# JuliaMolSim/Molly.jl

Hardware: AMD Instinct MI355X
Metric: ns_per_day (higher is better)
Workload: dtype f32; 1 GPU; 1M-atom LJ fluid (argon, rho=21.1/nm3), cubic PBC, DistanceCutoff 1.0 nm, r_list 1.2 nm, dt 2 fs, VelocityVerlet, remove_CM_motion=1; integrator=vv, n_atoms=1000000, rebuild_every=10, parallelism=single domain, block_atoms=256, j_split=2, pairs_half_list=75841147

## Files before the change

molly.jl_amd/csrc/kernels.h:

```cpp
#pragma once
#include <type_traits>
#include "pass_plan.h"
#include "physics.h"
#include "halo_xfer.h"
#include "philox.h"

namespace mhip {

enum { FLAG_MINIMG = 0, FLAG_OVERFLOW = 1, FLAG_MAX_TILE = 2, FLAG_MAX_ROWS = 3, FLAG_NAN = 4, FLAG_TOTAL_ROWS = 5, FLAG_MAX_CELLS = 6, FLAG_MAX_DISP2 = 7, FLAG_MAX_V2 = 8, N_FLAGS = 10 };
enum { OVF_TILE = 1, OVF_ROWS = 2, OVF_BOXCELLS = 4, OVF_SLOT = 8 };

constexpr int MAX_BOX_CELLS = 8192;
constexpr uint32_t XL_EXCLUDED = 1u << 30, XL_SPECIAL = 1u << 31, XL_INDEX = (1u << 30) - 1u;

constexpr int SLOT_MAX_SCALED = 16383;
__host__ __device__ inline uint32_t entry_slot(uint32_t e, int sh) { return sh ? (e >> sh) : (e & 0x7fffu); }
__host__ __device__ inline uint32_t entry_special(uint32_t e, int sh) { return sh ? 0u : (e >> 15); }
__host__ __device__ inline uint32_t make_entry(uint32_t slot, uint32_t sp, int sh) { return sh ? (slot << sh) : (slot | (sp << 15)); }

template <class T> __device__ inline int cell_coord(T x, int d, const GridP<T>& G) {
    T rel = G.periodic[d] ? x : x - G.origin[d];
    int c = (int)M<T>::floor(rel * G.inv_cs[d]);
    return min(max(c, 0), G.nc[d] - 1);
}
// ... 1039 lines not shown
[[maybe_unused]] static __device__ inline void halo_tail(const HaloStep& H, const double* cm_part, int n_part) {
    const int lane = threadIdx.x & 63;
    double a[4] = {0, 0, 0, 0};
    if (cm_part) for (int q = lane; q < n_part; q += 64) for (int c = 0; c < 4; ++c) a[c] += __hip_atomic_load(&cm_part[4 * (int64_t)q + c], __ATOMIC_RELAXED, __HIP_MEMORY_SCOPE_AGENT);
#pragma unroll
    for (int o = 32; o > 0; o >>= 1) for (int c = 0; c < 4; ++c) a[c] += __shfl_xor(a[c], o, 64);
    if (lane < 4) H.cm_all[lane] = lane == 0 ? a[0] : lane == 1 ? a[1] : lane == 2 ? a[2] : a[3];
    for (int q = lane; q < H.n_peers * H.cm_rows; q += 64) {
        const int r = q % H.cm_rows;
        float* d = H.cm_dst[q] + (int64_t)H.parity_send * H.half_stride;
        for (int c = 0; c < 3; ++c) {
            const int i = 3 * r + c;
            const unsigned long long bits = (unsigned long long)__double_as_longlong(i < 2 ? a[0] : i < 4 ? a[1] : i < 6 ? a[2] : a[3]);
            const float w = i < 8 ? __uint_as_float((uint32_t)((i & 1) ? bits >> 32 : bits)) : 0.f;
            __hip_atomic_store(d + c, w, __ATOMIC_RELAXED, __HIP_MEMORY_SCOPE_SYSTEM);
        }
    }
    __threadfence_system();
    if (lane < H.n_peers) xfer_store_release(H.ann[lane] + (size_t)H.parity_send * XFER_MAX_RANKS, H.seq_send);
    if (lane == 0) __hip_atomic_store(H.done, 0u, __ATOMIC_RELAXED, __HIP_MEMORY_SCOPE_AGENT);
}

template <class T> struct ForceArgs {
    GridP<T> G;
    InterP<T> I;
    int64_t n_owned;
    int BI, BI_shift, JS, T_cap, T_lds, R_cap, n_blocks, blocks_per_xcd;
    const typename Vec<T>::T4* pos;
    const typename Vec<T>::T2* lj;
    const int32_t* tile_idx;
    const int32_t* tile_cnt;
    const uint2* nbr;
    const int32_t* wave_rows;
    const typename Vec<T>::T4* blk_center;
    typename Vec<T>::T4* frc;
    double* pe_part;
    uint2* nbr_dst; int32_t* rows_dst; const typename Vec<T>::T4* pos_snap; float* blk_disp2; T r_prune2;
    int32_t* tile_idx_dst; int32_t* tile_cnt_dst; int mark_off;
    typename Vec<T>::T4* snap_dst;
    int any_special;
    int soa;
    int eshift;
    uint16_t* cnt_dst;
    const int32_t* blk_ghost; int part;
    int level_pairs;
    unsigned long long* dbg;
    const double* cm_fin_in; int cm_fin_n; double* cm_fin_out;
    typename Vec<T>::T4* vel; typename Vec<T>::T4* pos_next; T dt, dt2;
    const double* cm_in; int cm_n; unsigned long long* cm_pub; uint32_t step_seq; double* cm_out;
    float* trk_part; const typename Vec<T>::T4* snap_a; const typename Vec<T>::T4* snap_b;
    HaloStep H;
    const int32_t* orig; StochP<T> S;
};
[[maybe_unused]] static __device__ inline void step_cm_publish(const double* __restrict__ part, int n_part, unsigned long long* pub, uint32_t seq, unsigned char* smem) {
    double (*sh_pub)[4] = reinterpret_cast<double (*)[4]>(smem);
    double a[4] = {0, 0, 0, 0};
    for (int q = threadIdx.x; q < n_part; q += blockDim.x) { const double* p = part + 4 * (int64_t)q; a[0] += p[0]; a[1] += p[1]; a[2] += p[2]; a[3] += p[3]; }
#pragma unroll
    for (int o = 32; o > 0; o >>= 1) for (int c = 0; c < 4; ++c) a[c] += __shfl_xor(a[c], o, 64);
    if ((threadIdx.x & 63) == 0) for (int c = 0; c < 4; ++c) sh_pub[threadIdx.x >> 6][c] = a[c];
    __syncthreads();
    if (threadIdx.x < 3) {
        double t = 0, m = 0;
        for (int q = 0; q < (int)(blockDim.x >> 6); ++q) { t += sh_pub[q][threadIdx.x]; m += sh_pub[q][3]; }
        const float vc = (float)(t / m);
        __hip_atomic_store(&pub[threadIdx.x], (unsigned long long)__float_as_uint(vc) | ((unsigned long long)seq << 32), __ATOMIC_RELAXED, __HIP_MEMORY_SCOPE_AGENT);
    }
}
[[maybe_unused]] static __device__ inline void cm_finalize_in_block(const double* __restrict__ part, int n_part, double* out4, unsigned char* smem) {
    double a[4] = {0, 0, 0, 0};
    for (int q = threadIdx.x; q < n_part; q += blockDim.x) { const double* p = part + 4 * (int64_t)q; a[0] += p[0]; a[1] += p[1]; a[2] += p[2]; a[3] += p[3]; }
#pragma unroll
    for (int o = 32; o > 0; o >>= 1) for (int c = 0; c < 4; ++c) a[c] += __shfl_xor(a[c], o, 64);
    double* sh = reinterpret_cast<double*>(smem);
    if ((threadIdx.x & 63) == 0) for (int c = 0; c < 4; ++c) sh[4 * (threadIdx.x >> 6) + c] = a[c];
    __syncthreads();
    if (threadIdx.x < 4) { double t = 0; for (int q = 0; q < (int)(blockDim.x >> 6); ++q) t += sh[4 * q + threadIdx.x]; out4[threadIdx.x] = t; }
    __syncthreads();
}

#ifndef MHIP_FAST_MIN_WAVES
#define MHIP_FAST_MIN_WAVES 8
#endif
#ifndef MHIP_SB
#define MHIP_SB 4
#endif
template <class T, int LJM, int COULM, bool ENERGY, bool MINIMG, bool SEG, bool PRUNE>
constexpr int force_min_waves() { return (std::is_same<T, float>::value && LJM == LJ_DIST_UNIFORM && COULM == MHIP_COUL_NONE && !ENERGY && !MINIMG && !SEG && !PRUNE) ? MHIP_FAST_MIN_WAVES : 1; }

template <class T, int LJM, int COULM, bool ENERGY, bool MINIMG, bool SEG, bool PRUNE, int SOA_STRIDE = 4097, bool STEP = false, bool HALO = false, bool LANG = false>
__global__ void __launch_bounds__(BlockLimits<T>::max_threads, (force_min_waves<T, LJM, COULM, ENERGY, MINIMG, SEG, PRUNE>()))
k_forces(ForceArgs<T> A) {
    static_assert(!HALO || (STEP && std::is_same<T, float>::value), "the ghosted form exists for the fused fp32 step only");
    static_assert(!LANG || (STEP && !HALO), "the Langevin update rides in the fused single-domain step only");
    using T4 = typename Vec<T>::T4;
    using T2 = typename Vec<T>::T2;
    constexpr bool PER_ATOM_LJ = (LJM == LJ_DIST || LJM == LJ_GENERIC);
    extern __shared__ __align__(32) unsigned char smem[];
    const GridP<T>& G = A.G;
    int wg = blockIdx.x;
    if constexpr (STEP) {
        if (wg == 0) {
            if constexpr (HALO) { if (A.cm_in) halo_cm_publish(A.H, A.cm_pub, A.step_seq, smem); }
            else if (A.cm_in) step_cm_publish(A.cm_in, A.cm_n, A.cm_pub, A.step_seq, smem);
            return;
        }
        --wg;
    }
    int b = (wg & 7) * A.blocks_per_xcd + (wg >> 3);
    [[maybe_unused]] int hflags = 0;
    if constexpr (HALO) { b = A.H.order[wg]; if (b < 0) return; hflags = A.H.flags[b]; }
    else {
        if (b >= A.n_blocks) return;
        if (A.part != 0 && (A.blk_ghost[b] != 0) != (A.part == 2)) return;
    }
    const int tid = threadIdx.x, nthr = blockDim.x;
    [[maybe_unused]] auto stamp = [&](int k) {
        if constexpr (MHIP_STAMPS != 0 && !PRUNE) {
            if (A.dbg && (tid & 63) == 0) { unsigned long long* d = A.dbg + ((size_t)b * (nthr >> 6) + (tid >> 6)) * 8; d[k] = __builtin_readcyclecounter(); d[4 + k] = wall_clock64(); }
        }
    };
    stamp(0);
    const int tile_n = A.tile_cnt[b];
    T4* l_pos = reinterpret_cast<T4*>(smem);
    T2* l_lj = reinterpret_cast<T2*>(l_pos + (A.T_lds + 1));
    const T4 ctr = A.blk_center[b];
    constexpr bool MAY_SCALE = std::is_same<T, float>::value && LJM == LJ_DIST_UNIFORM && COULM == MHIP_COUL_NONE;
    const int esh = MAY_SCALE ? A.eshift : 0;

    auto localise = [&](T4 p, auto tri_tag) -> T4 {
        if constexpr (!MINIMG) local_xyz_t<decltype(tri_tag)::value>(p.x, p.y, p.z, ctr, G);
        return p;
    };
    constexpr bool NO_TRI = std::is_same<T, float>::value && LJM == LJ_DIST_UNIFORM && COULM == MHIP_COUL_NONE && !ENERGY;
    const bool tri_local = !MINIMG && !NO_TRI && G.tri_grid;
    const int li = tid & (A.BI - 1), js = tid >> A.BI_shift;
    const int64_t si = (int64_t)b * A.BI + li;
    const bool valid = si < A.n_owned;
    [[maybe_unused]] auto step_lane = [&]() -> int { int t = tid; asm volatile("" : "+v"(t)); return t & (A.BI - 1); };
    [[maybe_unused]] auto step_atom = [&]() -> int64_t { return (int64_t)b * A.BI + step_lane(); };
    T4 pi_raw;
    if constexpr (PRUNE || COULM != MHIP_COUL_NONE) pi_raw = A.pos[valid ? si : (int64_t)b * A.BI];
    else {
        const T* own = reinterpret_cast<const T*>(A.pos + (valid ? si : (int64_t)b * A.BI));
        pi_raw = make4<T>(own[0], own[1], own[2], T(0));
    }
    T4 pi;
    T2 lji_raw = make2<T>(T(0), T(0)), lji = lji_raw;
    if constexpr (PER_ATOM_LJ) lji_raw = A.lj[valid ? si : (int64_t)b * A.BI];
    constexpr bool PRE_E = PER_ATOM_LJ && sizeof(T) == 4;
    auto pre_e = [](T2 v) { if constexpr (PRE_E) { v.y = v.x == T(0) ? T(0) : M<T>::sqrt(v.y); v.x *= T(0.5); } return v; };
    const int rows_lane = A.wave_rows[(b * A.JS + js) * (A.BI >> 6) + (li >> 6)];
    int rows = 0;
    bool own_done = false;
    auto own_ready = [&]() {
        if (own_done) return;
        own_done = true;
        if constexpr (NO_TRI) pi = localise(pi_raw, std::false_type{});
        else pi = tri_local ? localise(pi_raw, std::true_type{}) : localise(pi_raw, std::false_type{});
        lji = pre_e(lji_raw);
        rows = __builtin_amdgcn_readfirstlane(rows_lane);
    };
    if constexpr (PRUNE) own_ready();
    const uint2* my_rows = A.nbr + (((int64_t)b * A.JS + js) * A.R_cap) * A.BI + li;
    const int32_t* tix = (HALO ? A.H.tsrc : A.tile_idx) + (int64_t)b * A.T_cap;
    if constexpr (HALO) { if (hflags & 1) halo_wait_block(A.H); }
    T fx = T(0), fy = T(0), fz = T(0), pe = T(0);
    [[maybe_unused]] T vir[6] = {T(0), T(0), T(0), T(0), T(0), T(0)};
    uint64_t acc = 0;
    int kept = 0;
    uint2* out_rows = nullptr;
    if constexpr (PRUNE) out_rows = A.nbr_dst + (((int64_t)b * A.JS + js) * A.R_cap) * A.BI + li;
    [[maybe_unused]] uint16_t* l_new = nullptr; [[maybe_unused]] int32_t* l_scan = nullptr; [[maybe_unused]] float* l_box = nullptr;
    [[maybe_unused]] int32_t* l_cnt = nullptr; [[maybe_unused]] int32_t* l_wmax = nullptr; [[maybe_unused]] const uint2* l_lut = nullptr;
    [[maybe_unused]] int n_new = 0;
    if constexpr (PRUNE) {
        l_new = reinterpret_cast<uint16_t*>(smem + A.mark_off);
        l_scan = reinterpret_cast<int32_t*>(smem + A.mark_off + ((A.T_lds + 8) & ~7) * 2);
        l_box = reinterpret_cast<float*>(l_scan + nthr + 4);
        l_wmax = reinterpret_cast<int32_t*>(l_box + 64); l_cnt = l_wmax + 64;
        if (tid < 64) l_wmax[tid] = 0;
        l_lut = reinterpret_cast<const uint2*>(l_cnt + nthr);
        if (tid < 16) {
            uint32_t sel[2] = {0x0c0c0c0cu, 0x0c0c0c0cu};
            int p = 0;
            for (int j = 0; j < 4; ++j) if ((tid >> j) & 1) {
                const int sh = (p & 1) * 16;
                sel[p >> 1] = (sel[p >> 1] & ~(0xffffu << sh)) | ((uint32_t)((2 * j) | ((2 * j + 1) << 8)) << sh);
                ++p;
            }
            reinterpret_cast<uint2*>(l_cnt + nthr)[tid] = make_uint2(sel[0], sel[1]);
        }
        const int lpb = A.BI >> 3;
        float mn[3] = {(float)pi.x, (float)pi.y, (float)pi.z}, mx[3] = {(float)pi.x, (float)pi.y, (float)pi.z};
        for (int o = lpb >> 1; o > 0; o >>= 1)
#pragma unroll
            for (int d = 0; d < 3; ++d) { mn[d] = fminf(mn[d], __shfl_xor(mn[d], o, WAVE)); mx[d] = fmaxf(mx[d], __shfl_xor(mx[d], o, WAVE)); }
        if (js == 0 && (li & (lpb - 1)) == 0) {
            reinterpret_cast<float4*>(l_box)[(li / lpb) * 2] = make_float4(mn[0], mn[1], mn[2], 0.f);
            reinterpret_cast<float4*>(l_box)[(li / lpb) * 2 + 1] = make_float4(mx[0], mx[1], mx[2], 0.f);
        }
        if (A.snap_dst && js == 0 && valid) A.snap_dst[si] = pi_raw;
    }
    [[maybe_unused]] auto emit4 = [&](uint32_t n0, uint32_t n1, uint32_t n2, uint32_t n3, bool k0, bool k1, bool k2, bool k3) {
        const uint32_t m = (k0 ? 1u : 0u) | (k1 ? 2u : 0u) | (k2 ? 4u : 0u) | (k3 ? 8u : 0u);
        const uint2 sel = l_lut[m];
        const uint32_t x = __builtin_amdgcn_perm(n1, n0, 0x05040100u), y = __builtin_amdgcn_perm(n3, n2, 0x05040100u);
        const uint64_t p = ((uint64_t)__builtin_amdgcn_perm(y, x, sel.y) << 32) | __builtin_amdgcn_perm(y, x, sel.x);
        const int np = kept & 3, sh = np * 16;
        const uint64_t c_lo = acc | (p << sh), c_hi = (p >> 1) >> (63 - sh);
        const int cnt = __builtin_popcount(m);
        const bool flush = np + cnt >= 4;
        if (flush) out_rows[(int64_t)(kept >> 2) * A.BI] = make_uint2((uint32_t)c_lo, (uint32_t)(c_lo >> 32));
        acc = flush ? c_hi : c_lo;
        kept += cnt;
    };
    auto emit = [&](uint32_t e) {
        const int np = kept & 3;
        acc |= (uint64_t)e << (np * 16);
        if (np == 3) { out_rows[(int64_t)(kept >> 2) * A.BI] = make_uint2((uint32_t)acc, (uint32_t)(acc >> 32)); acc = 0; }
        ++kept;
    };

    constexpr bool FAST_CT = std::is_same<T, float>::value && LJM == LJ_DIST_UNIFORM && COULM == MHIP_COUL_NONE && !ENERGY && !MINIMG && !SEG;
    const int seg_cap = A.T_lds;
    for (int seg_lo = 0; seg_lo < (SEG ? tile_n : 1); seg_lo += seg_cap) {
        const int n_here = SEG ? min(seg_cap, tile_n - seg_lo) : tile_n;
        if (SEG && seg_lo > 0) __syncthreads();
        const bool packed3 = FAST_CT && !A.any_special && A.soa == SOA_STRIDE && A.eshift == ESHIFT_SCALED;
        float* l_p3 = reinterpret_cast<float*>(smem);
        auto stage = [&](auto tri_tag) {
            constexpr int SB = (FAST_CT && !PRUNE) ? MHIP_SB : 4;
            if constexpr (FAST_CT && !PRUNE) {
                auto round = [&](int t0) {
                    int s[SB]; T4 p[SB];
#pragma unroll
                    for (int k = 0; k < SB; ++k) s[k] = tix[min(t0 + k * nthr + tid, A.T_cap - 1)];
#pragma unroll
                    for (int k = 0; k < SB; ++k) {
                        s[k] = (t0 + k * nthr + tid < n_here) ? s[k] : (int)((int64_t)b * A.BI);
                        if constexpr (HALO) {
                            if (s[k] >= 0) p[k] = A.pos[s[k]];
                            else { const float* gr = A.H.rows + 3 * (size_t)(-1 - s[k]); p[k] = make4<T>((T)peer_row_load(gr), (T)peer_row_load(gr + 1), (T)peer_row_load(gr + 2), T(0)); }
                        } else p[k] = A.pos[s[k]];
                    }
#pragma unroll
                    for (int k = 0; k < SB; ++k) {
                        const int t = t0 + k * nthr + tid;
                        if (t < n_here) {
                            const T4 pl = localise(p[k], tri_tag);
                            if (packed3) { l_p3[t] = (float)pl.x; l_p3[SOA_STRIDE + t] = (float)pl.y; l_p3[2 * SOA_STRIDE + t] = (float)pl.z; }
                            else l_pos[t] = pl;
                        }
                    }
                };
                round(0);
                for (int t0 = SB * nthr; t0 < n_here; t0 += SB * nthr) round(t0);
                return;
            }
            for (int t0 = 0; t0 < n_here; t0 += SB * nthr) {
                int s[SB]; T4 p[SB]; [[maybe_unused]] T2 q[SB];
                constexpr bool GUARD = !(FAST_CT && !PRUNE);
                const int kmax = GUARD ? min(SB, (n_here - t0 + nthr - 1) / nthr) : SB;
#pragma unroll
                for (int k = 0; k < SB; ++k) {
                    if (k < kmax) {
                        const int t = min(t0 + k * nthr + tid, n_here - 1);
                        s[k] = tix[seg_lo + t];
                    }
                }
#pragma unroll
                for (int k = 0; k < SB; ++k) if (k < kmax) { p[k] = A.pos[s[k]]; if constexpr (PER_ATOM_LJ) q[k] = A.lj[s[k]]; }
#pragma unroll
                for (int k = 0; k < SB; ++k) {
                    const int t = t0 + k * nthr + tid;
                    if (k < kmax && t < n_here) {
                        const T4 pl = localise(p[k], tri_tag);
                        if (packed3) { l_p3[t] = (float)pl.x; l_p3[SOA_STRIDE + t] = (float)pl.y; l_p3[2 * SOA_STRIDE + t] = (float)pl.z; }
                        else l_pos[t] = pl;
                        if constexpr (PER_ATOM_LJ) l_lj[t] = pre_e(q[k]);
                    }
                }
            }
        };
        if constexpr (NO_TRI) stage(std::false_type{});
        else { if (tri_local) stage(std::true_type{}); else stage(std::false_type{}); }
        own_ready();
        if (tid == 0) {
            if (packed3) { l_p3[n_here] = 1e4f; l_p3[SOA_STRIDE + n_here] = 1e4f; l_p3[2 * SOA_STRIDE + n_here] = 1e4f; }
            else l_pos[n_here] = make4<T>(T(1e4), T(1e4), T(1e4), T(0));
            if constexpr (PER_ATOM_LJ) l_lj[n_here] = make2<T>(T(0), T(0));
        }
        __syncthreads();
        if constexpr (PRUNE) {
            constexpr int NW = 8;
            const float reach2 = (float)A.r_prune2 * 1.001f + 1e-12f;
            const float bL[3] = {(float)G.L[0], (float)G.L[1], (float)G.L[2]}, biL[3] = {(float)G.invL[0], (float)G.invL[1], (float)G.invL[2]};
            auto stays = [&](int t) -> bool {
                if constexpr (MINIMG) { if (G.triclinic) return true; }
                float p[3];
                if (packed3) { p[0] = l_p3[t]; p[1] = l_p3[SOA_STRIDE + t]; p[2] = l_p3[2 * SOA_STRIDE + t]; }
                else { const T4 q = l_pos[t]; p[0] = (float)q.x; p[1] = (float)q.y; p[2] = (float)q.z; }
                float best = 3.0e38f;
#pragma unroll 1
                for (int w = 0; w < NW; ++w) {
                    const float4 lo = reinterpret_cast<const float4*>(l_box)[2 * w], hi = reinterpret_cast<const float4*>(l_box)[2 * w + 1];
                    float ex, ey, ez;
                    if constexpr (MINIMG) {
                        const float blo[3] = {lo.x, lo.y, lo.z}, bhi[3] = {hi.x, hi.y, hi.z};
                        float e[3];
#pragma unroll
                        for (int d = 0; d < 3; ++d) {
                            float dd = p[d] - 0.5f * (blo[d] + bhi[d]);
                            if (G.periodic[d]) dd -= bL[d] * rintf(dd * biL[d]);
                            e[d] = fmaxf(fabsf(dd) - 0.5f * (bhi[d] - blo[d]) - 1e-5f * bL[d], 0.f);
                        }
                        ex = e[0]; ey = e[1]; ez = e[2];
                    } else {
                        ex = fmaxf(fmaxf(lo.x - p[0], p[0] - hi.x), 0.f); ey = fmaxf(fmaxf(lo.y - p[1], p[1] - hi.y), 0.f); ez = fmaxf(fmaxf(lo.z - p[2], p[2] - hi.z), 0.f);
                    }
                    best = fminf(best, ex * ex + ey * ey + ez * ez);
                }
                return best <= reach2;
            };
            const int per = (n_here + nthr - 1) / nthr, t0 = min(tid * per, n_here), t1 = min(t0 + per, n_here);
            int cnt = 0;
            uint32_t keep_bits = 0;
            for (int t = t0; t < t1; ++t) { const bool k = stays(t); cnt += k ? 1 : 0; if (t - t0 < 32) keep_bits |= (k ? 1u : 0u) << (t - t0); }
            l_scan[tid] = cnt;
            __syncthreads();
            if (tid < WAVE) {
                int run = 0;
                for (int base = 0; base < nthr; base += WAVE) {
                    int v = (base + tid < nthr) ? l_scan[base + tid] : 0, x = v;
#pragma unroll
                    for (int o = 1; o < WAVE; o <<= 1) { int u = __shfl_up(x, o, WAVE); if (tid >= o) x += u; }
                    if (base + tid < nthr) l_scan[base + tid] = run + x - v;
                    run += __shfl(x, WAVE - 1, WAVE);
                }
                if (tid == 0) l_scan[nthr] = run;
            }
            __syncthreads();
            {
                int run = n_new + l_scan[tid];
                for (int t = t0; t < t1; ++t) {
                    if ((t - t0 < 32) ? ((keep_bits >> (t - t0)) & 1u) != 0u : stays(t)) { l_new[t] = (uint16_t)(packed3 ? run << ESHIFT_SCALED : run); A.tile_idx_dst[(int64_t)b * A.T_cap + run] = tix[seg_lo + t]; ++run; }
                    else l_new[t] = (uint16_t)0xffffu;
                }
            }
            n_new += l_scan[nthr];
            __syncthreads();
        }
        stamp(1);
        auto walk_rows = [&](auto spec_tag) {
            constexpr bool SPEC = decltype(spec_tag)::value;
            if constexpr (FAST_CT && !SPEC) { if (packed3) {
                typedef float v2f __attribute__((ext_vector_type(2)));
                const v2f pix = {(float)pi.x, (float)pi.x}, piy = {(float)pi.y, (float)pi.y}, piz = {(float)pi.z, (float)pi.z};
                const float c6 = (float)A.I.lj_c6, c12 = (float)A.I.lj_c12, rc2 = (float)A.I.lj_rc2, rp2 = (float)A.r_prune2;
                const float rc2n = __int_as_float(__float_as_int(rc2) + 1);
                const v2f cut_a = {-0x1p100f, -0x1p100f}, cut_b = {rc2n * 0x1p100f, rc2n * 0x1p100f};
                const v2f c48v = {c12, c12}, c24v = {c6, c6};
                v2f fx2 = {(float)fx, 0.f}, fy2 = {(float)fy, 0.f}, fz2 = {(float)fz, 0.f};
                typedef __attribute__((address_space(3))) const char* lds_cptr;
                const lds_cptr lbase = (lds_cptr)(uintptr_t)0;
                auto lds3 = [&](uint32_t oa, uint32_t ob, v2f& dx, v2f& dy, v2f& dz) {
                    typedef __attribute__((address_space(3))) const float* lds_fptr;
                    const lds_fptr pa = (lds_fptr)(lbase + oa), pb = (lds_fptr)(lbase + ob);
                    dx = (v2f){pa[0], pb[0]} - pix; dy = (v2f){pa[SOA_STRIDE], pb[SOA_STRIDE]} - piy; dz = (v2f){pa[2 * SOA_STRIDE], pb[2 * SOA_STRIDE]} - piz;
                };
                auto row = [&](const uint2 e4) {
                    const uint32_t oa = e4.x & 0xffffu, ob = e4.x >> 16, oc = e4.y & 0xffffu, od = e4.y >> 16;
                    v2f dx0, dy0, dz0, dx1, dy1, dz1;
                    lds3(oa, ob, dx0, dy0, dz0); lds3(oc, od, dx1, dy1, dz1);
                    __builtin_amdgcn_sched_group_barrier(0x100, 12, 0);
                    const v2f r20 = __builtin_elementwise_fma(dz0, dz0, __builtin_elementwise_fma(dy0, dy0, dx0 * dx0));
                    const v2f r21 = __builtin_elementwise_fma(dz1, dz1, __builtin_elementwise_fma(dy1, dy1, dx1 * dx1));
                    if constexpr (PRUNE) {
                        typedef __attribute__((address_space(3))) const unsigned short* lds_hptr;
                        auto new_entry = [&](uint32_t o) -> uint32_t { return (uint32_t)*(lds_hptr)(lbase + prune_mark_ct(SOA_STRIDE) + (o >> 1)); };
                        const uint32_t na = new_entry(oa), nb = new_entry(ob), nc = new_entry(oc), nd = new_entry(od);
                        emit4(na, nb, nc, nd, r20.x <= rp2, r20.y <= rp2, r21.x <= rp2, r21.y <= rp2);
                    }
                    const float t0 = __builtin_amdgcn_rcpf(r20.x * r20.y), t1 = __builtin_amdgcn_rcpf(r21.x * r21.y);
                    const v2f u0 = (v2f){r20.y, r20.x} * t0, u1 = (v2f){r21.y, r21.x} * t1;
                    v2f in0, in1;
                    asm("v_pk_fma_f32 %0, %1, %2, %3 clamp\n\ts_nop 0" : "=v"(in0) : "v"(r20), "s"(cut_a), "v"(cut_b));
                    asm("v_pk_fma_f32 %0, %1, %2, %3 clamp\n\ts_nop 0" : "=v"(in1) : "v"(r21), "s"(cut_a), "v"(cut_b));
                    const v2f q0 = u0 * u0, q1 = u1 * u1;
                    const v2f w0 = u0 * in0, w1 = u1 * in1;
                    const v2f c0 = q0 * u0, c1 = q1 * u1;
                    const v2f g0 = __builtin_elementwise_fma(c0, c48v, -c24v), g1 = __builtin_elementwise_fma(c1, c48v, -c24v);
                    const v2f h0 = c0 * w0, h1 = c1 * w1;
                    const v2f f0 = g0 * h0, f1 = g1 * h1;
                    fx2 -= dx0 * f0; fy2 -= dy0 * f0; fz2 -= dz0 * f0;
                    fx2 -= dx1 * f1; fy2 -= dy1 * f1; fz2 -= dz1 * f1;
                };
                if (rows > 0) {
                    const int last = rows - 1;
                    constexpr int D = 2;
                    uint2 e[D] = {my_rows[0], my_rows[(int64_t)min(1, last) * A.BI]};
                    auto next = [&](int q) -> uint2 { return my_rows[(int64_t)min(q, last) * A.BI]; };
                    int r = 0;
                    for (; r + D <= rows; r += D) {
#pragma unroll
                        for (int k = 0; k < D; ++k) { row(e[k]); e[k] = next(r + D + k); }
                    }
#pragma unroll
                    for (int k = 0; k < D - 1; ++k) if (r + k < rows) row(e[k]);
                }
                fx = (T)(fx2.x + fx2.y); fy = (T)(fy2.x + fy2.y); fz = (T)(fz2.x + fz2.y);
                return;
            } }
            constexpr bool PK2 = std::is_same<T, float>::value && LJM == LJ_DIST && (COULM == MHIP_COUL_EWALD_DIRECT || COULM == MHIP_COUL_REACTION_FIELD) && !ENERGY;
            [[maybe_unused]] bool pk2_ok = false;
            if constexpr (PK2) pk2_ok = Pk2Consts::usable(reinterpret_cast<const InterP<float>&>(A.I));
            [[maybe_unused]] auto row_pk2 = [&](const uint2 e4) {
                if constexpr (PK2) {
                    const Pk2Consts K(A.I);
                    const float kqi = (float)A.I.ke * (float)pi.w, si = (float)lji.x, ei24 = 24.f * (float)lji.y;
                    v2f fxy = {0.f, 0.f}; float fzs = 0.f;
#pragma unroll
                    for (int h = 0; h < 2; ++h) {
                        const uint32_t ew = h ? e4.y : e4.x;
                        uint32_t sa = ew & 0x7fffu, sb = (ew >> 16) & 0x7fffu;
                        [[maybe_unused]] const bool real_a = SEG ? (sa - (uint32_t)seg_lo) < (uint32_t)n_here : sa < (uint32_t)tile_n, real_b = SEG ? (sb - (uint32_t)seg_lo) < (uint32_t)n_here : sb < (uint32_t)tile_n;
                        if constexpr (SEG) { sa = real_a ? sa - (uint32_t)seg_lo : (uint32_t)n_here; sb = real_b ? sb - (uint32_t)seg_lo : (uint32_t)n_here; }
                        float4 pa, pb; float2 la, lb;
                        pa = *reinterpret_cast<const float4*>(&l_pos[sa]); pb = *reinterpret_cast<const float4*>(&l_pos[sb]);
                        la = *reinterpret_cast<const float2*>(&l_lj[sa]); lb = *reinterpret_cast<const float2*>(&l_lj[sb]);
                        v2f da, db; float dza, dzb;
                        if constexpr (MINIMG) {
                            float x, y, z;
                            min_image_exact<float>((float)pi.x, (float)pi.y, (float)pi.z, pa.x, pa.y, pa.z, reinterpret_cast<const GridP<float>&>(G), x, y, z); da = (v2f){x, y}; dza = z;
                            min_image_exact<float>((float)pi.x, (float)pi.y, (float)pi.z, pb.x, pb.y, pb.z, reinterpret_cast<const GridP<float>&>(G), x, y, z); db = (v2f){x, y}; dzb = z;
                        } else {
                            const v2f pixy = {(float)pi.x, (float)pi.y};
                            da = (v2f){pa.x, pa.y} - pixy; db = (v2f){pb.x, pb.y} - pixy; dza = pa.z - (float)pi.z; dzb = pb.z - (float)pi.z;
                        }
                        const v2f qa = da * da, qb = db * db;
                        v2f r2 = {__builtin_fmaf(dza, dza, qa.x + qa.y), __builtin_fmaf(dzb, dzb, qb.x + qb.y)};
                        if constexpr (MINIMG) { if (G.triclinic) { if (!real_a) r2.x = 1.0e12f; if (!real_b) r2.y = 1.0e12f; } }
                        if constexpr (PRUNE) {
                            if (valid && real_a && r2.x <= (float)A.r_prune2) emit(make_entry((uint32_t)l_new[sa], 0u, 0));
                            if (valid && real_b && r2.y <= (float)A.r_prune2) emit(make_entry((uint32_t)l_new[sb], 0u, 0));
                        }
                        const v2f fr = pair_eval2<COULM>(reinterpret_cast<const InterP<float>&>(A.I), K, r2, kqi, (v2f){pa.w, pb.w}, si, (v2f){la.x, lb.x}, ei24, (v2f){la.y, lb.y});
                        fxy += da * (v2f){fr.x, fr.x}; fxy += db * (v2f){fr.y, fr.y};
                        fzs = __builtin_fmaf(dza, fr.x, __builtin_fmaf(dzb, fr.y, fzs));
                    }
                    fx -= (T)fxy.x; fy -= (T)fxy.y; fz -= (T)fzs;
                }
            };
            uint2 e_next = (0 < rows) ? my_rows[0] : make_uint2(0, 0);
            constexpr int UNROLL = (sizeof(T) == 8 && (COULM == MHIP_COUL_EWALD_DIRECT || COULM == COUL_EWALD_EXACT)) ? (MINIMG ? 1 : (LJM == LJ_GENERIC && ENERGY ? 2 : 4)) : 4;
            for (int r = 0; r < rows; ++r) {
                const uint2 e4 = e_next;
                if (r + 1 < rows) e_next = my_rows[(int64_t)(r + 1) * A.BI];
                if constexpr (PK2) {
                    if (pk2_ok && (!SPEC || __builtin_amdgcn_ballot_w64(((e4.x | e4.y) & 0x80008000u) != 0u) == 0ull)) { row_pk2(e4); continue; }
                }
#pragma unroll UNROLL
                for (int k = 0; k < 4; ++k) {
                    uint32_t e = ((k < 2 ? e4.x : e4.y) >> (16 * (k & 1))) & 0xffffu;
                    uint32_t slot = entry_slot(e, esh);
                    [[maybe_unused]] const bool real = SEG ? (slot - (uint32_t)seg_lo) < (uint32_t)n_here : slot < (uint32_t)tile_n;
                    if constexpr (SEG) { slot -= (uint32_t)seg_lo; slot = slot < (uint32_t)n_here ? slot : (uint32_t)n_here; }
                    const bool special = SPEC ? entry_special(e, esh) != 0 : false;
                    T4 pj = l_pos[slot];
                    T2 ljj = make2<T>(T(0), T(0));
                    if constexpr (PER_ATOM_LJ) ljj = l_lj[slot];
                    T dx, dy, dz;
                    if constexpr (MINIMG) {
                        min_image_exact<T>(pi.x, pi.y, pi.z, pj.x, pj.y, pj.z, G, dx, dy, dz);
                    } else { dx = pj.x - pi.x; dy = pj.y - pi.y; dz = pj.z - pi.z; }
                    T r2 = dx * dx + dy * dy + dz * dz;
                    if constexpr (MINIMG) { if (G.triclinic && !real) r2 = T(1.0e30); }
                    if constexpr (PRUNE) { if (real && valid && r2 <= A.r_prune2) emit(make_entry((uint32_t)l_new[slot], entry_special(e, esh), esh)); }
                    T fr = pair_eval<T, LJM, COULM, ENERGY, PRE_E>(A.I, r2, pi.w, pj.w, lji.x, ljj.x, lji.y, ljj.y, special, pe);
                    fx -= fr * dx; fy -= fr * dy; fz -= fr * dz;
                    if constexpr (ENERGY) {
                        vir[0] += fr * dx * dx; vir[1] += fr * dy * dy; vir[2] += fr * dz * dz;
                        vir[3] += fr * dx * dy; vir[4] += fr * dx * dz; vir[5] += fr * dy * dz;
                    }
                }
            }
        };
        if constexpr (LJM == LJ_DIST_UNIFORM && COULM == MHIP_COUL_NONE && !ENERGY) {
            if (A.any_special) walk_rows(std::true_type{}); else walk_rows(std::false_type{});
        } else walk_rows(std::true_type{});
        if constexpr (!SEG) break;
    }
    if constexpr (PRUNE) {
        const uint32_t SENTP = make_entry((uint32_t)n_new, 0u, esh);
        const int NWB = A.BI >> 6;
        const bool level = A.level_pairs && A.JS == 2;
        if (level) {
            if (kept & 3) out_rows[(int64_t)(kept >> 2) * A.BI] = make_uint2((uint32_t)acc, (uint32_t)(acc >> 32));
            l_cnt[tid] = kept;
            __syncthreads();
            const int kp = l_cnt[tid ^ A.BI], total = kept + kp, mine = js == 0 ? (total + 1) >> 1 : total >> 1;
            if (kept > mine) {
                uint16_t* to = reinterpret_cast<uint16_t*>(A.nbr_dst + (((int64_t)b * A.JS + (js ^ 1)) * A.R_cap) * A.BI + li);
                const uint16_t* from = reinterpret_cast<const uint16_t*>(out_rows);
                for (int q = 0; q < kept - mine; ++q) {
                    const int ps = mine + q, pd = kp + q;
                    to[(((int64_t)(pd >> 2) * A.BI) << 2) + (pd & 3)] = from[(((int64_t)(ps >> 2) * A.BI) << 2) + (ps & 3)];
                }
            }
            kept = mine;
        }
        if (A.cnt_dst) A.cnt_dst[((int64_t)b * A.JS + js) * A.BI + li] = (uint16_t)min(kept, 65535);
        atomicMax(&l_wmax[js * NWB + (li >> 6)], (kept + 3) >> 2);
        __syncthreads();
        const int rows_wave = l_wmax[js * NWB + (li >> 6)];
        if (level) {
            uint16_t* mine16 = reinterpret_cast<uint16_t*>(out_rows);
            for (int p2 = kept; p2 < 4 * rows_wave; ++p2) mine16[(((int64_t)(p2 >> 2) * A.BI) << 2) + (p2 & 3)] = (uint16_t)SENTP;
        } else
        while (((kept + 3) >> 2) < rows_wave || (kept & 3)) emit(SENTP);
        if (tid < A.JS * NWB) A.rows_dst[b * A.JS * NWB + tid] = l_wmax[tid];
        if (tid == 0) A.tile_cnt_dst[b] = n_new;
        float d2 = 0.f;
        if (valid && js == 0) {
            T4 q = A.pos_snap[si];
            T ex = pi_raw.x - q.x, ey = pi_raw.y - q.y, ez = pi_raw.z - q.z;
            disp_image(ex, ey, ez, G);
            d2 = (float)(ex * ex + ey * ey + ez * ez);
        }
        d2 = wave_max(d2);
        if (js == 0 && (tid & 63) == 0) A.blk_disp2[b * (A.BI >> 6) + (li >> 6)] = d2;
    }
    stamp(2);
    [[maybe_unused]] T4 st_v, st_p;
    [[maybe_unused]] int64_t se = 0;
    [[maybe_unused]] unsigned long long st_w[3] = {0, 0, 0};
    [[maybe_unused]] int snd0 = 0, snd1 = 0;
    if constexpr (STEP) {
        __builtin_amdgcn_s_setprio(3);
        se = step_atom();
        if constexpr (HALO) { if ((hflags & 2) && js == 0 && se < A.n_owned) { snd0 = A.H.snd_start[se]; snd1 = A.H.snd_start[se + 1]; } }
        if (js == 0 && se < A.n_owned) {
            st_v = A.vel[se]; st_p = A.pos[se];
            if (A.cm_in) {
#pragma unroll
                for (int c = 0; c < 3; ++c) st_w[c] = __hip_atomic_load(&A.cm_pub[c], __ATOMIC_RELAXED, __HIP_MEMORY_SCOPE_AGENT);
            }
        }
    }
    if (A.JS > 1) {
        __syncthreads();
        T* red = reinterpret_cast<T*>(smem);
        red[(js * 4 + 0) * A.BI + li] = fx; red[(js * 4 + 1) * A.BI + li] = fy;
        red[(js * 4 + 2) * A.BI + li] = fz; red[(js * 4 + 3) * A.BI + li] = pe;
        __syncthreads();
        if (js == 0) {
            for (int q = 1; q < A.JS; ++q) {
                fx += red[(q * 4 + 0) * A.BI + li]; fy += red[(q * 4 + 1) * A.BI + li];
                fz += red[(q * 4 + 2) * A.BI + li]; pe += red[(q * 4 + 3) * A.BI + li];
            }
        }
    }
    if constexpr (STEP) {
        double px = 0, py = 0, pz = 0, pm = 0;
        float tr_a = 0.f, tr_b = 0.f, tr_v = 0.f;
        T4 v = st_v, p = st_p;
        const bool mine = js == 0 && se < A.n_owned;
        if (mine) {
            if (A.cm_in) {
                if constexpr (HALO) {
                    if ((uint32_t)(st_w[0] >> 32) != A.step_seq || (uint32_t)(st_w[1] >> 32) != A.step_seq || (uint32_t)(st_w[2] >> 32) != A.step_seq) {
                        __builtin_amdgcn_s_setprio(0);
                        const unsigned long long t0 = wall_clock64();
                        do {
                            __builtin_amdgcn_s_sleep(16);
#pragma unroll
                            for (int c = 0; c < 3; ++c) st_w[c] = __hip_atomic_load(&A.cm_pub[c], __ATOMIC_RELAXED, __HIP_MEMORY_SCOPE_AGENT);
                        } while (((uint32_t)(st_w[0] >> 32) != A.step_seq || (uint32_t)(st_w[1] >> 32) != A.step_seq || (uint32_t)(st_w[2] >> 32) != A.step_seq) && wall_clock64() - t0 < 2 * A.H.ticks);
                        __builtin_amdgcn_s_setprio(3);
                    }
                } else
                while ((uint32_t)(st_w[0] >> 32) != A.step_seq || (uint32_t)(st_w[1] >> 32) != A.step_seq || (uint32_t)(st_w[2] >> 32) != A.step_seq) {
#pragma unroll
                    for (int c = 0; c < 3; ++c) st_w[c] = __hip_atomic_load(&A.cm_pub[c], __ATOMIC_RELAXED, __HIP_MEMORY_SCOPE_AGENT);
                }
                T vc[3];
#pragma unroll
                for (int c = 0; c < 3; ++c) vc[c] = (T)__uint_as_float((uint32_t)st_w[c]);
                v.x -= vc[0]; v.y -= vc[1]; v.z -= vc[2];
                if constexpr (!LANG) { p.x = M<T>::sub(p.x, M<T>::mul(vc[0], A.dt)); p.y = M<T>::sub(p.y, M<T>::mul(vc[1], A.dt)); p.z = M<T>::sub(p.z, M<T>::mul(vc[2], A.dt)); }
            }
            if constexpr (LANG) {
                const T4 f4 = make4<T>(fx, fy, fz, T(0));
                langevin_atom<T>(v, p, f4, A.S, (uint64_t)A.orig[se] + 1, G);
                if (A.cm_out) { px = (double)v.x * v.w; py = (double)v.y * v.w; pz = (double)v.z * v.w; pm = v.w; }
            } else {
            const T kx = M<T>::mul(accel_of(fx, v.w), A.dt2), ky = M<T>::mul(accel_of(fy, v.w), A.dt2), kz = M<T>::mul(accel_of(fz, v.w), A.dt2);
            v.x = M<T>::add(v.x, kx); v.y = M<T>::add(v.y, ky); v.z = M<T>::add(v.z, kz);
            if (A.cm_out) { px = (double)v.x * v.w; py = (double)v.y * v.w; pz = (double)v.z * v.w; pm = v.w; }
            v.x = M<T>::add(v.x, kx); v.y = M<T>::add(v.y, ky); v.z = M<T>::add(v.z, kz);
            p.x = step_add(p.x, v.x, A.dt); p.y = step_add(p.y, v.y, A.dt); p.z = step_add(p.z, v.z, A.dt);
            wrap_point(p.x, p.y, p.z, G);
            }
            if (A.trk_part) {
                tr_v = (float)(v.x * v.x + v.y * v.y + v.z * v.z);
                auto q = A.snap_a[se];
// ... 187 lines not shown
```

molly.jl_amd/csrc/pass_plan.h:

```cpp
#pragma once
#include <algorithm>
#include <cstddef>
#include <cstdint>

#include "../../include/mollyhip.h"

#if defined(__HIPCC__) || defined(__CUDACC__)
#define MHIP_PLAN_HD __host__ __device__
#else
#define MHIP_PLAN_HD
#endif

namespace mhip {

constexpr int MAX_LDS_BYTES = 160 * 1024 - 2048;
enum { LJ_OFF = 0, LJ_DIST = 1, LJ_GENERIC = 2, LJ_DIST_UNIFORM = 3 };
constexpr int ESHIFT_SCALED = 2;

constexpr int SOA_STRIDES[3] = {2049, 3073, 4097};
MHIP_PLAN_HD constexpr int lds_align16(int bytes) { return (bytes + 15) & ~15; }
MHIP_PLAN_HD constexpr int packed_tile_bytes(int soa) { return 3 * soa * 4 + 64; }
MHIP_PLAN_HD constexpr int prune_mark_ct(int soa) { return lds_align16(packed_tile_bytes(soa)); }
MHIP_PLAN_HD inline size_t prune_lds_bytes(int t_seg, int nthr) { return (size_t)(((t_seg + 8) & ~7) * 2) + ((size_t)nthr + 4) * 4 + 8 * 8 * 4 + ((size_t)nthr + 64) * 4 + 16 * 8 + 32; }

inline size_t gs_lds_bytes(int q_lds, int BI, int JSW) { return std::max((size_t)(q_lds + 1) * (16 + 8), (size_t)JSW * 3 * BI * 4) + 64; }
inline int regroup_list_bytes(int BI, int JS, int R_cap) { return (int)std::min<size_t>((size_t)MAX_LDS_BYTES - (size_t)JS * BI * 16 - 64, (size_t)JS * R_cap * BI * 8); }

inline size_t block_reduction_bytes(int BI, int JS, size_t real) { return (size_t)JS * 4 * BI * real; }
inline size_t tile_record_bytes(bool per_atom_lj, size_t real) { return 4 * real + (per_atom_lj ? 2 * real : 0); }
inline size_t force_lds_bytes(int t_lds, int BI, int JS, bool per_atom_lj, size_t real) {
    return std::max(std::max((size_t)(t_lds + 1) * tile_record_bytes(per_atom_lj, real), block_reduction_bytes(BI, JS, real)), (size_t)BI * sizeof(double)) + 32;
}
struct TileCarve { bool segmented; int t_lds; size_t bytes; };
inline TileCarve carve_tile(int tile_max, size_t budget, size_t reserve, int BI, int JS, bool per_atom_lj, size_t real) {
    budget = std::min<size_t>(budget, MAX_LDS_BYTES);
    if (budget > reserve + 8192) budget -= reserve;
    const size_t per_atom = tile_record_bytes(per_atom_lj, real);
    const size_t fixed = std::max(block_reduction_bytes(BI, JS, real), (size_t)BI * sizeof(double)) + 64;
    int fit = (int)((budget > fixed + 2 * per_atom ? budget - fixed : 2 * per_atom) / per_atom) - 1;
    fit = std::max(fit & ~1, 2);
    TileCarve c;
    c.segmented = tile_max > fit;
    c.t_lds = c.segmented ? fit : std::max(tile_max, 1);
    c.bytes = force_lds_bytes(c.t_lds, BI, JS, per_atom_lj, real);
    return c;
}

struct PassShape {
    bool fp32 = true; int ljm = LJ_OFF, coulm = MHIP_COUL_NONE;
    bool minimg = false; int n_special = 0, eshift = 0; bool lj_c12 = false;
    int BI = 64, JS = 1, T_cap = 16;
    size_t lds_budget = MAX_LDS_BYTES;
    bool dual = false, inner_valid = false;
    int max_tile = 0, max_tile_in = 0;
    int gs = 0; bool gs_list_current = false;
    int64_t n_ghost = 0;
    bool energy = false; int part = 0;
    bool allow_gs = false, own_frc = false;
    bool step = false, halo = false, fuse_step = true;
    int cm_mode = 0, cm_n = 0; bool in_step_loop = false;
};

enum class PassForm { GROUP_SPLIT, PACKED, GENERIC };
enum class PassCapacity { OK, TILE, PRUNE };
struct PassPlan {
    PassForm form = PassForm::GENERIC;
    bool prune = false, use_inner = false;
    int tile_max = 0;
    bool segmented = false; int tile_lds = 0;
    int soa = 0;
    size_t lds_bytes = 0;
    int mark_off = 0;
    int q_lds = 0;
    bool can_step = false;
    bool steps = false;
    bool cm_slot = false;
    bool cm_fin = false;
    PassCapacity capacity = PassCapacity::OK;
    int tile_segments() const { return segmented ? (std::max(tile_max, 1) + std::max(tile_lds, 1) - 1) / std::max(tile_lds, 1) : 1; }
};
inline const char* capacity_message(PassCapacity c) {
    return c == PassCapacity::TILE ? "force-kernel LDS carve-up exceeds 160 KiB" : c == PassCapacity::PRUNE ? "prune pass LDS carve-up exceeds 160 KiB" : "";
}

inline bool packed_kind(const PassShape& s) {
    return s.fp32 && s.ljm == LJ_DIST_UNIFORM && s.coulm == MHIP_COUL_NONE && !s.energy && !s.minimg && s.n_special == 0 && s.eshift == ESHIFT_SCALED && s.lj_c12;
}
inline int packed_stride(int tile_max) {
    for (int k = 0; k < 3; ++k) if (tile_max + 1 < SOA_STRIDES[k]) return SOA_STRIDES[k];
    return 0;
}

inline void plan_tile(PassPlan& p, const PassShape& s, int tile_max, size_t reserve = 0) {
    const size_t real = s.fp32 ? sizeof(float) : sizeof(double);
    const TileCarve c = carve_tile(tile_max, s.lds_budget, reserve, s.BI, s.JS, s.ljm == LJ_DIST || s.ljm == LJ_GENERIC, real);
    p.tile_max = tile_max; p.segmented = c.segmented; p.tile_lds = c.t_lds; p.lds_bytes = c.bytes;
    if (c.bytes > (size_t)MAX_LDS_BYTES) p.capacity = PassCapacity::TILE;
}

inline PassPlan plan_pass(const PassShape& s) {
    PassPlan p;
    p.use_inner = s.dual && s.inner_valid;
    p.prune = s.dual && !s.inner_valid && !s.energy;
    p.tile_max = p.use_inner ? s.max_tile_in : s.max_tile;
    const bool whole = !s.energy && s.part == 0 && !s.own_frc;
    auto hand_over = [&] {
// ... 32 lines not shown
```

Baseline: 1339 ns/day.

## Raise prune-pass occupancy, use scalar row bases, and swizzle LDS tile slots

The fp32 uniform-LJ prune variant of the force kernel now gets a min-waves launch bound of 6 instead of 1. Neighbour-row pointers become wave-uniform scalar bases with per-lane byte offsets, which saves vector registers, and the displacement check reads atoms by step index. Packed LDS tile slots are also permuted by an XOR on one bit, applied both when staging and when decoding entries, to spread LDS bank accesses. The occupancy target can force register spills, and the swizzle adds ALU work to every row decode.

After: 1335 ns/day, median of 2. No clear change (-0.3%).

```diff
diff --git a/molly.jl_amd/csrc/kernels.h b/molly.jl_amd/csrc/kernels.h
--- a/molly.jl_amd/csrc/kernels.h
+++ b/molly.jl_amd/csrc/kernels.h
@@ -1145,11 +1145,14 @@
 #ifndef MHIP_FAST_MIN_WAVES
 #define MHIP_FAST_MIN_WAVES 8
 #endif
+#ifndef MHIP_PRUNE_MIN_WAVES
+#define MHIP_PRUNE_MIN_WAVES 6
+#endif
 #ifndef MHIP_SB
 #define MHIP_SB 4
 #endif
 template <class T, int LJM, int COULM, bool ENERGY, bool MINIMG, bool SEG, bool PRUNE>
-constexpr int force_min_waves() { return (std::is_same<T, float>::value && LJM == LJ_DIST_UNIFORM && COULM == MHIP_COUL_NONE && !ENERGY && !MINIMG && !SEG && !PRUNE) ? MHIP_FAST_MIN_WAVES : 1; }
+constexpr int force_min_waves() { return (std::is_same<T, float>::value && LJM == LJ_DIST_UNIFORM && COULM == MHIP_COUL_NONE && !ENERGY && !MINIMG && !SEG) ? (PRUNE ? MHIP_PRUNE_MIN_WAVES : MHIP_FAST_MIN_WAVES) : 1; }
 
 template <class T, int LJM, int COULM, bool ENERGY, bool MINIMG, bool SEG, bool PRUNE, int SOA_STRIDE = 4097, bool STEP = false, bool HALO = false, bool LANG = false>
 __global__ void __launch_bounds__(BlockLimits<T>::max_threads, (force_min_waves<T, LJM, COULM, ENERGY, MINIMG, SEG, PRUNE>()))
@@ -1225,7 +1228,13 @@
         rows = __builtin_amdgcn_readfirstlane(rows_lane);
     };
     if constexpr (PRUNE) own_ready();
-    const uint2* my_rows = A.nbr + (((int64_t)b * A.JS + js) * A.R_cap) * A.BI + li;
+    constexpr bool LEAN = PRUNE && force_min_waves<T, LJM, COULM, ENERGY, MINIMG, SEG, PRUNE>() > 1;
+    const int js_u = LEAN ? __builtin_amdgcn_readfirstlane(js) : js;
+    const uint2* my_rows = A.nbr + (((int64_t)b * A.JS + js_u) * A.R_cap) * A.BI + (LEAN ? 0 : li);
+    auto in_row = [&](int q) -> uint2 {
+        if constexpr (LEAN) return *reinterpret_cast<const uint2*>(reinterpret_cast<const char*>(my_rows + (int64_t)q * A.BI) + ((uint32_t)li << 3));
+        else return my_rows[(int64_t)q * A.BI];
+    };
     const int32_t* tix = (HALO ? A.H.tsrc : A.tile_idx) + (int64_t)b * A.T_cap;
     if constexpr (HALO) { if (hflags & 1) halo_wait_block(A.H); }
     T fx = T(0), fy = T(0), fz = T(0), pe = T(0);
@@ -1233,7 +1242,11 @@
     uint64_t acc = 0;
     int kept = 0;
     uint2* out_rows = nullptr;
-    if constexpr (PRUNE) out_rows = A.nbr_dst + (((int64_t)b * A.JS + js) * A.R_cap) * A.BI + li;
+    if constexpr (PRUNE) out_rows = A.nbr_dst + (((int64_t)b * A.JS + js_u) * A.R_cap) * A.BI + (LEAN ? 0 : li);
+    [[maybe_unused]] auto put_row = [&](int row, uint2 v) {
+        if constexpr (LEAN) *reinterpret_cast<uint2*>(reinterpret_cast<char*>(out_rows) + ((((uint32_t)row << A.BI_shift) + (uint32_t)li) << 3)) = v;
+        else out_rows[(int64_t)row * A.BI] = v;
+    };
     [[maybe_unused]] uint16_t* l_new = nullptr; [[maybe_unused]] int32_t* l_scan = nullptr; [[maybe_unused]] float* l_box = nullptr;
     [[maybe_unused]] int32_t* l_cnt = nullptr; [[maybe_unused]] int32_t* l_wmax = nullptr; [[maybe_unused]] const uint2* l_lut = nullptr;
     [[maybe_unused]] int n_new = 0;
@@ -1274,14 +1287,14 @@
         const uint64_t c_lo = acc | (p << sh), c_hi = (p >> 1) >> (63 - sh);
         const int cnt = __builtin_popcount(m);
         const bool flush = np + cnt >= 4;
-        if (flush) out_rows[(int64_t)(kept >> 2) * A.BI] = make_uint2((uint32_t)c_lo, (uint32_t)(c_lo >> 32));
+        if (flush) put_row(kept >> 2, make_uint2((uint32_t)c_lo, (uint32_t)(c_lo >> 32)));
         acc = flush ? c_hi : c_lo;
         kept += cnt;
     };
     auto emit = [&](uint32_t e) {
         const int np = kept & 3;
         acc |= (uint64_t)e << (np * 16);
-        if (np == 3) { out_rows[(int64_t)(kept >> 2) * A.BI] = make_uint2((uint32_t)acc, (uint32_t)(acc >> 32)); acc = 0; }
+        if (np == 3) { put_row(kept >> 2, make_uint2((uint32_t)acc, (uint32_t)(acc >> 32))); acc = 0; }
         ++kept;
     };
 
@@ -1292,6 +1305,8 @@
         if (SEG && seg_lo > 0) __syncthreads();
         const bool packed3 = FAST_CT && !A.any_special && A.soa == SOA_STRIDE && A.eshift == ESHIFT_SCALED;
         float* l_p3 = reinterpret_cast<float*>(smem);
+        constexpr int SWZ_BIT = (PRUNE && FAST_CT) ? PRUNE_SWZ_BIT : 0;
+        [[maybe_unused]] auto tau = [&](int t) -> int { return (SWZ_BIT != 0 && packed3) ? prune_tile_index(t, SWZ_BIT) : t; };
         auto stage = [&](auto tri_tag) {
             constexpr int SB = (FAST_CT && !PRUNE) ? MHIP_SB : 4;
             if constexpr (FAST_CT && !PRUNE) {
@@ -1339,7 +1354,7 @@
                     const int t = t0 + k * nthr + tid;
                     if (k < kmax && t < n_here) {
                         const T4 pl = localise(p[k], tri_tag);
-                        if (packed3) { l_p3[t] = (float)pl.x; l_p3[SOA_STRIDE + t] = (float)pl.y; l_p3[2 * SOA_STRIDE + t] = (float)pl.z; }
+                        if (packed3) { const int ts = tau(t); l_p3[ts] = (float)pl.x; l_p3[SOA_STRIDE + ts] = (float)pl.y; l_p3[2 * SOA_STRIDE + ts] = (float)pl.z; }
                         else l_pos[t] = pl;
                         if constexpr (PER_ATOM_LJ) l_lj[t] = pre_e(q[k]);
                     }
@@ -1350,7 +1365,7 @@
         else { if (tri_local) stage(std::true_type{}); else stage(std::false_type{}); }
         own_ready();
         if (tid == 0) {
-            if (packed3) { l_p3[n_here] = 1e4f; l_p3[SOA_STRIDE + n_here] = 1e4f; l_p3[2 * SOA_STRIDE + n_here] = 1e4f; }
+            if (packed3) { const int ts = tau(n_here); l_p3[ts] = 1e4f; l_p3[SOA_STRIDE + ts] = 1e4f; l_p3[2 * SOA_STRIDE + ts] = 1e4f; }
             else l_pos[n_here] = make4<T>(T(1e4), T(1e4), T(1e4), T(0));
             if constexpr (PER_ATOM_LJ) l_lj[n_here] = make2<T>(T(0), T(0));
         }
@@ -1362,7 +1377,7 @@
             auto stays = [&](int t) -> bool {
                 if constexpr (MINIMG) { if (G.triclinic) return true; }
                 float p[3];
-                if (packed3) { p[0] = l_p3[t]; p[1] = l_p3[SOA_STRIDE + t]; p[2] = l_p3[2 * SOA_STRIDE + t]; }
+                if (packed3) { const int ts = tau(t); p[0] = l_p3[ts]; p[1] = l_p3[SOA_STRIDE + ts]; p[2] = l_p3[2 * SOA_STRIDE + ts]; }
                 else { const T4 q = l_pos[t]; p[0] = (float)q.x; p[1] = (float)q.y; p[2] = (float)q.z; }
                 float best = 3.0e38f;
 #pragma unroll 1
@@ -1407,8 +1422,8 @@
             {
                 int run = n_new + l_scan[tid];
                 for (int t = t0; t < t1; ++t) {
-                    if ((t - t0 < 32) ? ((keep_bits >> (t - t0)) & 1u) != 0u : stays(t)) { l_new[t] = (uint16_t)(packed3 ? run << ESHIFT_SCALED : run); A.tile_idx_dst[(int64_t)b * A.T_cap + run] = tix[seg_lo + t]; ++run; }
-                    else l_new[t] = (uint16_t)0xffffu;
+                    if ((t - t0 < 32) ? ((keep_bits >> (t - t0)) & 1u) != 0u : stays(t)) { l_new[tau(t)] = (uint16_t)(packed3 ? run << ESHIFT_SCALED : run); A.tile_idx_dst[(int64_t)b * A.T_cap + run] = tix[seg_lo + t]; ++run; }
+                    else l_new[tau(t)] = (uint16_t)0xffffu;
                 }
             }
             n_new += l_scan[nthr];
@@ -1432,7 +1447,8 @@
                     const lds_fptr pa = (lds_fptr)(lbase + oa), pb = (lds_fptr)(lbase + ob);
                     dx = (v2f){pa[0], pb[0]} - pix; dy = (v2f){pa[SOA_STRIDE], pb[SOA_STRIDE]} - piy; dz = (v2f){pa[2 * SOA_STRIDE], pb[2 * SOA_STRIDE]} - piz;
                 };
-                auto row = [&](const uint2 e4) {
+                auto row = [&](uint2 e4) {
+                    if constexpr (SWZ_BIT != 0) { e4.x = prune_tile_word(e4.x, SWZ_BIT); e4.y = prune_tile_word(e4.y, SWZ_BIT); }
                     const uint32_t oa = e4.x & 0xffffu, ob = e4.x >> 16, oc = e4.y & 0xffffu, od = e4.y >> 16;
                     v2f dx0, dy0, dz0, dx1, dy1, dz1;
                     lds3(oa, ob, dx0, dy0, dz0); lds3(oc, od, dx1, dy1, dz1);
@@ -1462,8 +1478,8 @@
                 if (rows > 0) {
                     const int last = rows - 1;
                     constexpr int D = 2;
-                    uint2 e[D] = {my_rows[0], my_rows[(int64_t)min(1, last) * A.BI]};
-                    auto next = [&](int q) -> uint2 { return my_rows[(int64_t)min(q, last) * A.BI]; };
+                    uint2 e[D] = {LEAN ? in_row(0) : my_rows[0], in_row(min(1, last))};
+                    auto next = [&](int q) -> uint2 { return in_row(min(q, last)); };
                     int r = 0;
                     for (; r + D <= rows; r += D) {
 #pragma unroll
@@ -1515,11 +1531,11 @@
                     fx -= (T)fxy.x; fy -= (T)fxy.y; fz -= (T)fzs;
                 }
             };
-            uint2 e_next = (0 < rows) ? my_rows[0] : make_uint2(0, 0);
+            uint2 e_next = (0 < rows) ? in_row(0) : make_uint2(0, 0);
             constexpr int UNROLL = (sizeof(T) == 8 && (COULM == MHIP_COUL_EWALD_DIRECT || COULM == COUL_EWALD_EXACT)) ? (MINIMG ? 1 : (LJM == LJ_GENERIC && ENERGY ? 2 : 4)) : 4;
             for (int r = 0; r < rows; ++r) {
                 const uint2 e4 = e_next;
-                if (r + 1 < rows) e_next = my_rows[(int64_t)(r + 1) * A.BI];
+                if (r + 1 < rows) e_next = in_row(r + 1);
                 if constexpr (PK2) {
                     if (pk2_ok && (!SPEC || __builtin_amdgcn_ballot_w64(((e4.x | e4.y) & 0x80008000u) != 0u) == 0ull)) { row_pk2(e4); continue; }
                 }
@@ -1559,13 +1575,13 @@
         const int NWB = A.BI >> 6;
         const bool level = A.level_pairs && A.JS == 2;
         if (level) {
-            if (kept & 3) out_rows[(int64_t)(kept >> 2) * A.BI] = make_uint2((uint32_t)acc, (uint32_t)(acc >> 32));
+            if (kept & 3) put_row(kept >> 2, make_uint2((uint32_t)acc, (uint32_t)(acc >> 32)));
             l_cnt[tid] = kept;
             __syncthreads();
             const int kp = l_cnt[tid ^ A.BI], total = kept + kp, mine = js == 0 ? (total + 1) >> 1 : total >> 1;
             if (kept > mine) {
                 uint16_t* to = reinterpret_cast<uint16_t*>(A.nbr_dst + (((int64_t)b * A.JS + (js ^ 1)) * A.R_cap) * A.BI + li);
-                const uint16_t* from = reinterpret_cast<const uint16_t*>(out_rows);
+                const uint16_t* from = reinterpret_cast<const uint16_t*>(out_rows + (LEAN ? li : 0));
                 for (int q = 0; q < kept - mine; ++q) {
                     const int ps = mine + q, pd = kp + q;
                     to[(((int64_t)(pd >> 2) * A.BI) << 2) + (pd & 3)] = from[(((int64_t)(ps >> 2) * A.BI) << 2) + (ps & 3)];
@@ -1578,13 +1594,22 @@
         __syncthreads();
         const int rows_wave = l_wmax[js * NWB + (li >> 6)];
         if (level) {
-            uint16_t* mine16 = reinterpret_cast<uint16_t*>(out_rows);
+            uint16_t* mine16 = reinterpret_cast<uint16_t*>(out_rows + (LEAN ? li : 0));
             for (int p2 = kept; p2 < 4 * rows_wave; ++p2) mine16[(((int64_t)(p2 >> 2) * A.BI) << 2) + (p2 & 3)] = (uint16_t)SENTP;
         } else
         while (((kept + 3) >> 2) < rows_wave || (kept & 3)) emit(SENTP);
         if (tid < A.JS * NWB) A.rows_dst[b * A.JS * NWB + tid] = l_wmax[tid];
         if (tid == 0) A.tile_cnt_dst[b] = n_new;
         float d2 = 0.f;
+        if constexpr (LEAN) {
+            const int64_t sd = step_atom();
+            if (sd < A.n_owned && js == 0) {
+                const T4 q = A.pos_snap[sd], pr = A.pos[sd];
+                T ex = pr.x - q.x, ey = pr.y - q.y, ez = pr.z - q.z;
+                disp_image(ex, ey, ez, G);
+                d2 = (float)(ex * ex + ey * ey + ez * ez);
+            }
+        } else
         if (valid && js == 0) {
             T4 q = A.pos_snap[si];
             T ex = pi_raw.x - q.x, ey = pi_raw.y - q.y, ez = pi_raw.z - q.z;
diff --git a/molly.jl_amd/csrc/pass_plan.h b/molly.jl_amd/csrc/pass_plan.h
--- a/molly.jl_amd/csrc/pass_plan.h
+++ b/molly.jl_amd/csrc/pass_plan.h
@@ -22,6 +22,13 @@
 MHIP_PLAN_HD constexpr int packed_tile_bytes(int soa) { return 3 * soa * 4 + 64; }
 MHIP_PLAN_HD constexpr int prune_mark_ct(int soa) { return lds_align16(packed_tile_bytes(soa)); }
 MHIP_PLAN_HD inline size_t prune_lds_bytes(int t_seg, int nthr) { return (size_t)(((t_seg + 8) & ~7) * 2) + ((size_t)nthr + 4) * 4 + 8 * 8 * 4 + ((size_t)nthr + 64) * 4 + 16 * 8 + 32; }
+#ifndef MHIP_PRUNE_SWZ_BIT
+#define MHIP_PRUNE_SWZ_BIT 5
+#endif
+constexpr int PRUNE_SWZ_BIT = MHIP_PRUNE_SWZ_BIT;
+static_assert(PRUNE_SWZ_BIT >= 0 && PRUNE_SWZ_BIT <= 11, "the flip bit is a slot bit: entries are 16-bit byte offsets, slot << 2, of tiles below 4096 slots");
+MHIP_PLAN_HD constexpr int prune_tile_index(int t, int bit = PRUNE_SWZ_BIT) { return bit ? t ^ ((t >> bit) & 1) : t; }
+MHIP_PLAN_HD constexpr uint32_t prune_tile_word(uint32_t w, int bit = PRUNE_SWZ_BIT) { return bit ? w ^ ((w >> bit) & 0x00040004u) : w; }
 
 inline size_t gs_lds_bytes(int q_lds, int BI, int JSW) { return std::max((size_t)(q_lds + 1) * (16 + 8), (size_t)JSW * 3 * BI * 4) + 64; }
 inline int regroup_list_bytes(int BI, int JS, int R_cap) { return (int)std::min<size_t>((size_t)MAX_LDS_BYTES - (size_t)JS * BI * 16 - 64, (size_t)JS * R_cap * BI * 8); }
```
